# xiaolong-li1/VIDEO-BLADE

Hardware: AMD Instinct MI355X
Metric: frames/sec (aggregate over n_gpus; per GPU = value/n_gpus), CogVideoX-5B 8-step 49x720x480 bf16 (attention path); attn TFLOPS vs dense (higher is better)
Workload: dtype bf16; 1 GPU; CogVideoX-5B 8-step 49x720x480 bf16: 336 inner_attention calls per video (8 steps x 42 blocks), q/k/v [1,48,17776,64] (13x30x45 latent tokens + 226 text); global_batch=1, seq_len=17776, heads=48, head_dim=64, mask=energy rule (reference defaults), parallelism=replicas x1 (prompt-batch DP, no collective)

## Files before the change

include/vblade.h:

```cpp
#ifndef VBLADE_H_
#define VBLADE_H_

#include <stdint.h>

#ifdef __cplusplus
extern "C" {
#endif

#define VB_ABI_VERSION 4

#define VB_WORK_QUEUE_INTS 288

enum vb_status {
  VB_OK = 0,
  VB_ERR_INVALID = -1,
  VB_ERR_UNSUPPORTED = -2,
  VB_ERR_LAUNCH = -3
};

enum vb_dtype { VB_DTYPE_BF16 = 0, VB_DTYPE_F16 = 1 };
enum vb_mask_head_mode { VB_MASK_HEAD_PER_HEAD = 0, VB_MASK_HEAD_SHARED0 = 1 };

const char* vb_last_error(void);
int vb_abi_version(void);
// ... 71 lines not shown
int vb_mask_predict_long(const vb_predict_args* args, void* stream);

enum vb_rule_mode { VB_RULE_ENERGY = 0, VB_RULE_TOPK = 1 };
typedef struct vb_mask_rule {
  int mode;
  const int32_t* min_keep;
  const int32_t* max_keep;
  const float*   energy_threshold;
  int            init_k;
  const int32_t* init_k_bh;
  float          grow_below, shrink_below;
} vb_mask_rule;

int vb_mask_predict_rule(const vb_predict_args* args, const vb_mask_rule* rule, void* stream);

int vb_block_mask_rule(const void* po, int B, int H, int nr, int nc, const vb_mask_rule* rule,
                       float energy_threshold, int min_keep, int max_keep, int force_tail, int dtype,
                       uint8_t* mask, unsigned long long* mask_count, int32_t* rows_kept, void* stream);

int vb_sample_offsets(const float* rand_q, const float* rand_k, int rows, int n, int keep,
                      int32_t* q_off, int32_t* k_off, void* stream);

int vb_energy_mask(const void* po, int B, int H, int nr, int nc, float energy_threshold,
                   int min_keep, int max_keep, int force_tail, int dtype, uint8_t* mask,
                   unsigned long long* mask_count, void* stream);

int vb_pool_kv(const void* k, const void* v, const int64_t* k_stride, const int64_t* v_stride,
               const int32_t* rows, int B, int H, int L, int D, int gap, int dtype, void* kp,
               void* vp, void* k_r, void* v_r, void* stream);

// ... 223 lines not shown
```

video-blade_amd/csrc/vb_predict.hip:

```cpp
#include <cstdlib>

#include "vb_trace.hpp"

#ifndef VB_PRED_TRACE
#define VB_PRED_TRACE 0
#endif
#ifndef VB_PRED_STAMPS
#define VB_PRED_STAMPS 0
#endif
#if VB_PRED_TRACE
namespace vb { __device__ TraceBuf g_pred_trace; }
#define VB_TRACE_START(k) trace_start(g_pred_trace, k)
#define VB_TRACE_END() trace_end(g_pred_trace)
#endif
#if VB_PRED_STAMPS
namespace vb { __device__ unsigned long long g_pred_stamp[8]; }
#define VB_PRED_KERNEL_STAMPS 1
#endif

#include "vb_predict_kernel.hpp"

namespace vb {

__global__ void __launch_bounds__(256) topk_offsets_kernel(const float* rq, const float* rk, int rows, int n,
// ... 130 lines not shown
#endif
#if VB_PRED_STAMPS
extern "C" int vb_debug_pred_stamps(unsigned long long* out) {
  if (hipMemcpyFromSymbol(out, HIP_SYMBOL(vb::g_pred_stamp), 8 * sizeof(unsigned long long)) != hipSuccess) return -1;
  unsigned long long z[8] = {0, 0, 0, 0, 0, 0, 0, 0};
  return hipMemcpyToSymbol(HIP_SYMBOL(vb::g_pred_stamp), z, sizeof(z)) == hipSuccess ? 0 : -1;
}
#endif

extern "C" uint64_t vb_mask_predict_workspace_size(const vb_predict_args* a) {
  if (!a || a->B <= 0 || a->H <= 0 || a->L <= 0 || a->D <= 0 || a->num_keep <= 0) return 0;
  return vb::predict_ws_bytes(a->B, a->H, a->L, a->num_keep);
}

template <bool kLong>
static int mask_predict_entry(const vb_predict_args* a, void* stream, const vb_mask_rule* rule = nullptr) {
  using namespace vb;
  const std::string fn = rule ? "vb_mask_predict_rule: " : kLong ? "vb_mask_predict_long: " : "vb_mask_predict: ";
  if (!a || !a->q || !a->k || !a->q_off || !a->k_off || !a->po)
    return fail(VB_ERR_INVALID, fn + "null argument");
  if (a->B <= 0 || a->H <= 0 || a->L <= 0) return fail(VB_ERR_INVALID, fn + "bad sizes");
  if (a->block != 128 || (a->num_keep != 16 && a->num_keep != 32 && a->num_keep != 64))
    return fail(VB_ERR_UNSUPPORTED, fn + "block must be 128 and num_keep 16, 32 or 64 (got block " +
                                        std::to_string(a->block) + ", num_keep " + std::to_string(a->num_keep) + ")");
  const int nb = (a->L + a->block - 1) / a->block;
  if (nb > (kLong ? kMaxNbLong : kMaxNb)) return fail(VB_ERR_UNSUPPORTED, fn + "sequence too long");
  if (!kLong && a->L > 65535) return fail(VB_ERR_UNSUPPORTED, fn + "L must be < 65536");
  PredParams p{};
  if (rule) {
    if (a->mask_level) return fail(VB_ERR_INVALID, fn + "mask_level and a rule are exclusive");
    if (int rc = resolve_rule(rule, nb, a->min_keep, a->max_keep, fn, &p.rule)) return rc;
  } else if (a->min_keep < 1 || a->max_keep < 1) {
    return fail(VB_ERR_INVALID, fn + "keep counts must be >= 1");
// ... 30 lines not shown
    return fail(VB_ERR_INVALID, fn + "0..8 level bands with value/start/end arrays");
  if (a->mask_level) {
    if (!a->mask) return fail(VB_ERR_INVALID, fn + "mask_level needs a mask output");
    p.level = 1;
    p.lv.n = a->level_bands;
    for (int i = 0; i < a->level_bands; ++i) {
      const int val = a->level_band_value[i];
      if (val != 0 && val != 1 && val != 2 && val != 4 && val != 8)
        return fail(VB_ERR_INVALID, fn + "band values must be 0, 1, 2, 4 or 8");
      const int ia = (int)((double)nb * a->level_band_start[i]), ib = (int)((double)nb * a->level_band_end[i]);
      p.lv.value[i] = val;
      p.lv.start[i] = ia < 0 ? 0 : ia;
      p.lv.end[i] = ib > nb ? nb : ib;
    }
  }
  if (a->philox) {
    if (a->rand_q || a->rand_k) return fail(VB_ERR_INVALID, fn + "philox and rand_q/rand_k are exclusive");
    const int64_t one_pass = philox_x_only_numel();
    if (one_pass <= 0) return fail(VB_ERR_LAUNCH, fn + "cannot query the device's CU count");
    if ((int64_t)a->B * a->H * a->block > one_pass)
      return fail(VB_ERR_UNSUPPORTED, fn + "philox draws need B*H*block <= " + std::to_string(one_pass) +
                                          " (CUs x max threads per CU of this device)");
    p.philox = 1; p.philox_seed = a->philox_seed; p.philox_offset = a->philox_offset;
  }
  if (a->pool_kp) {
    if (!a->pool_v || !a->pool_vp || a->pool_gap <= 0 || ((a->pool_k_r == nullptr) != (a->pool_v_r == nullptr)))
      return fail(VB_ERR_INVALID, fn + "pool_v, pool_vp, pool_gap > 0 and both or neither of pool_k_r/pool_v_r");
    PoolTask& t = p.pool;
    t.D = a->D; t.gap = a->pool_gap;
    t.Lp = (a->L + a->pool_gap - 1) / a->pool_gap;
    if (int rc = fused_pass_setup(a, fn, t.Lp, t, &p.n_pool)) return rc;
    t.kp = reinterpret_cast<uint8_t*>(a->pool_kp); t.vp = reinterpret_cast<uint8_t*>(a->pool_vp);
    t.k_r = reinterpret_cast<uint8_t*>(a->pool_k_r); t.v_r = reinterpret_cast<uint8_t*>(a->pool_v_r);
  }
  if (a->pyr_k) {
    if (a->pool_kp) return fail(VB_ERR_INVALID, fn + "pool_* and pyr_* are exclusive");
    if (!a->pyr_v || !a->pool_v) return fail(VB_ERR_INVALID, fn + "pyr_k needs pyr_v and pool_v");
    PyrTask& t = p.pyr;
// ... 12 lines not shown
  hipEvent_t ev = reinterpret_cast<hipEvent_t>(a->staged_event);
  if (a->dtype != VB_DTYPE_BF16 && a->dtype != VB_DTYPE_F16) return fail(VB_ERR_INVALID, fn + "unknown dtype");
  return dispatch_predict<kLong>(p, a->dtype, a->num_keep, rule != nullptr, s, ev);
}

extern "C" int vb_mask_predict(const vb_predict_args* a, void* stream) { return mask_predict_entry<false>(a, stream); }

extern "C" int vb_mask_predict_long(const vb_predict_args* a, void* stream) {
  return mask_predict_entry<true>(a, stream);
}

extern "C" int vb_mask_predict_rule(const vb_predict_args* a, const vb_mask_rule* rule, void* stream) {
  if (rule) return mask_predict_entry<true>(a, stream, rule);
  if (a && a->block > 0 && a->L > 0 && (a->L + a->block - 1) / a->block > vb::kMaxNb) return mask_predict_entry<true>(a, stream);
  return mask_predict_entry<false>(a, stream);
}

extern "C" int vb_block_mask_rule(const void* po, int B, int H, int nr, int nc, const vb_mask_rule* rule,
                                  float energy_threshold, int min_keep, int max_keep, int force_tail, int dtype,
                                  uint8_t* mask, unsigned long long* mask_count, int32_t* rows_kept, void* stream) {
  using namespace vb;
  const std::string fn = "vb_block_mask_rule: ";
  if (!po || !mask) return fail(VB_ERR_INVALID, fn + "null argument");
  if (B <= 0 || H <= 0 || nr <= 0 || nc <= 0) return fail(VB_ERR_INVALID, fn + "bad sizes");
  if (nc > kMaxNbLong) return fail(VB_ERR_UNSUPPORTED, fn + "too many columns");
  if (force_tail < 0) return fail(VB_ERR_INVALID, fn + "force_tail must be >= 0");
  RuleParams rp{};
  vb_mask_rule none{};
  if (int rc = resolve_rule(rule ? rule : &none, nc, min_keep, max_keep, fn, &rp)) return rc;
  if (dtype != VB_DTYPE_BF16 && dtype != VB_DTYPE_F16) return fail(VB_ERR_INVALID, fn + "unknown dtype");
// ... 45 lines not shown
```

video-blade_amd/csrc/vb_predict_kernel.hpp:

```cpp
#pragma once
#include <type_traits>

#include <rocrand/rocrand_kernel.h>

#include "vb_tiles.hpp"
#include "vb_pool.hpp"
#include "vb_pyr.hpp"
#include "vb_mask_rows.hpp"

namespace vb {

constexpr int kPWaves = 4;
constexpr int kPThreads = 64 * kPWaves;
constexpr int kPMinWg = 2;
template <int D> constexpr int kKeysPerTile = (D == 64) ? 128 : 64;
template <int D> constexpr int kPBufs = D == 64 ? 2 : 3;

constexpr int kPSched = 4;
constexpr int kPRCols = 3;
typedef int i32x4 __attribute__((ext_vector_type(4)));
template <int D> constexpr bool kPoolLast = D == 128;
constexpr int kFusedPoolWgs = 320;
constexpr int kFusedPoolWgs64 = 384;

struct PredParams {
  const void* q; const void* k;
  int64_t qs[3], ks[3];
  void* reserved;
  int32_t* k_row_off;
  uint16_t* rbuf;
  const int32_t* rows;
  int32_t* q_off; int32_t* k_off;
  const float* rand_q; const float* rand_k;
  int philox; unsigned long long philox_seed, philox_offset;
  PoolTask pool;
  PyrTask pyr;
  int n_pool, pool_kind;
  int level;
  PredBands lv;
  int B, H, L, D, block, nb;
  float c;
  float thr;
  int min_keep, max_keep, force_tail;
  void* po;
  uint8_t* mask;
  unsigned long long* count;
  int32_t* rows_kept;
  int dbg;
  RuleParams rule;
};

#ifndef VB_DIAG
#define VB_DIAG 0
#endif
#ifndef VB_TRACE_START
#define VB_TRACE_START(k)
#define VB_TRACE_END()
#endif
#ifndef VB_PRED_KERNEL_STAMPS
#define VB_PRED_KERNEL_STAMPS 0
#endif
#if VB_PRED_KERNEL_STAMPS
__device__ __forceinline__ unsigned long long pred_stamp() {
  unsigned long long t;
// ... 50 lines not shown
      const float4 w = s4[j4];
      const int j = 4 * j4;
      rank += (w.x > v || (w.x == v && j < i)) ? 1 : 0;
      rank += (w.y > v || (w.y == v && j + 1 < i)) ? 1 : 0;
      rank += (w.z > v || (w.z == v && j + 2 < i)) ? 1 : 0;
      rank += (w.w > v || (w.w == v && j + 3 < i)) ? 1 : 0;
    }
    for (int j = 4 * n4; j < n; ++j) {
      const float w = sv[j];
      rank += (w > v || (w == v && j < i)) ? 1 : 0;
    }
    if (i < n && rank < keep) dst[rank] = i;
  }
}

template <class T, int kKeep = 32>
__global__ void __launch_bounds__(256) sample_rows_kernel(const PredParams p) {
  __shared__ alignas(16) float sv[2][256];
  __shared__ int32_t koff_s[kKeep];
  const int bh = blockIdx.y;
  const int wave = threadIdx.x >> 6;
  const int32_t* koff = p.k_off + (int64_t)bh * kKeep;
  if (p.philox) {
    if (wave == 0) {
      philox_draw_wave(p.philox_seed, p.philox_offset + 4, (long long)bh * p.block, p.block, sv[0]);
      topk_wave_lds(p.block, kKeep, koff_s, sv[0]);
    }
    if (blockIdx.x == 0 && wave == 1) {
      philox_draw_wave(p.philox_seed, p.philox_offset, (long long)bh * p.block, p.block, sv[1]);
      topk_wave_lds(p.block, kKeep, p.q_off + (int64_t)bh * kKeep, sv[1]);
    }
    __syncthreads();
    if (blockIdx.x == 0 && threadIdx.x < kKeep) p.k_off[(int64_t)bh * kKeep + threadIdx.x] = koff_s[threadIdx.x];
    koff = koff_s;
  } else if (p.rand_k) {
    if (wave == 0) topk_wave(p.rand_k + (int64_t)bh * p.block, p.block, kKeep, koff_s, sv[0]);
    if (blockIdx.x == 0 && wave == 1)
      topk_wave(p.rand_q + (int64_t)bh * p.block, p.block, kKeep, p.q_off + (int64_t)bh * kKeep, sv[1]);
    __syncthreads();
    if (blockIdx.x == 0 && threadIdx.x < kKeep) p.k_off[(int64_t)bh * kKeep + threadIdx.x] = koff_s[threadIdx.x];
    koff = koff_s;
  }
  const int jt = blockIdx.x * blockDim.x + threadIdx.x;
  if (jt >= p.nb * kKeep) return;
  constexpr int kKeepLog2 = kKeep == 16 ? 4 : kKeep == 32 ? 5 : 6;
  static_assert(kKeep == 1 << kKeepLog2, "sampling densities: 16, 32 or 64 tokens per block");
  int pos = min((jt >> kKeepLog2) * p.block + koff[jt & (kKeep - 1)], p.L - 1);
  if (p.rows) pos = p.rows[pos];
  p.k_row_off[(int64_t)bh * p.nb * kKeep + jt] =(int32_t)((int64_t)pos * p.ks[2] * 2);
}

template <int D, class T, bool kLong = false, int kKeep = 32, bool kRule = false>
__global__ void __launch_bounds__(kPThreads, kPMinWg) mask_predict_kernel(const PredParams p) {
  static_assert(!kRule || kLong, "the rule instantiations are long ones");
  static_assert(kKeep == 16 || kKeep == 32 || kKeep == 64, "sampling densities: 16, 32 or 64 tokens per block");
  constexpr int KS = D / 16;
  constexpr int kRowB = D * 2;
  constexpr int kKT = kKeysPerTile<D> / 32;
  constexpr int kTileBytes = kKeysPerTile<D> * kRowB;
  constexpr int kRowsPerInst = 1024 / kRowB;
  constexpr int kInstPerWave = kTileBytes / 1024 / kPWaves;
  constexpr int kBufs = kPBufs<D>;
  constexpr int KQ = 1;
  constexpr int kSt = kKeep == 16 ? kKT : KQ * (kKT / 2);
  const bool pool_wg = kPoolLast<D> ? (int)blockIdx.x >= (int)gridDim.x - p.n_pool : (int)blockIdx.x < p.n_pool;
  if (pool_wg) {
    VB_TRACE_START(1);
    const int pw = kPoolLast<D> ? (int)blockIdx.x - ((int)gridDim.x - p.n_pool) : (int)blockIdx.x;
    const int64_t i0 = (int64_t)pw * blockDim.x + threadIdx.x, st = (int64_t)p.n_pool * blockDim.x;
    if (p.pool_kind == 2) kv_pyramid_span<D, T>(p.pyr, i0, st);
    else pool_kv_span<T>(p.pool, i0, st);
    VB_TRACE_END();
    return;
  }
  VB_TRACE_START(0);
  const int wg = kPoolLast<D> ? (int)blockIdx.x : (int)blockIdx.x - p.n_pool;
  extern __shared__ __attribute__((aligned(16))) uint8_t smem[];
  const int nb = p.nb;
  float* mrow_s = reinterpret_cast<float*>(smem);
  uint8_t* ktile = smem + kPWaves * KQ * 32 * 4;
  float* rowbuf = reinterpret_cast<float*>(ktile);
  static_assert(kPWaves * 2 * kERow<kLong> * 4 <= kBufs * kTileBytes + 4 * kPWaves * 256,
                "the per-wave row scratch must fit in the K-tile ring it overlays");

  const int lane = threadIdx.x & 63;
  const int wave = __builtin_amdgcn_readfirstlane(threadIdx.x >> 6);
  const int half = lane >> 5;
  const int l32 = lane & 31;
  const int ng = kKeep == 64 ? 2 * nb : kKeep == 16 ? (nb + 1) >> 1 : nb;
  const int nqg = (ng + kPWaves * KQ - 1) / (kPWaves * KQ);
  const int lin = xcd_linear(wg, nqg * p.B * p.H);
  const int bh = lin / nqg;
// ... 319 lines not shown
  const size_t tiles = D == 64 ? (size_t)kPBufs<64> * kKeysPerTile<64> * 64 * 2
                               : (size_t)kPBufs<128> * kKeysPerTile<128> * 128 * 2;
  const size_t scratch = (size_t)kPWaves * 2 * (long_rows ? kEnergyRowLong : kEnergyRow) * 4;
  const size_t ring = 4 * kPWaves * 256;
  const size_t mrow = (size_t)kPWaves * 32 * 4;
  return mrow + (tiles + ring > scratch ? tiles + ring : scratch);
}

template <int D, class T, bool kLong, int kKeep = 32, bool kRule = false>
static int launch_predict(const PredParams& p, hipStream_t stream, hipEvent_t staged) {
  const size_t smem = predict_smem_bytes(D, kLong);
  auto kern = mask_predict_kernel<D, T, kLong, kKeep, kRule>;
  if (hipFuncSetAttribute(reinterpret_cast<const void*>(kern), hipFuncAttributeMaxDynamicSharedMemorySize,
                          (int)smem) != hipSuccess)
    return fail(VB_ERR_LAUNCH, "mask_predict: cannot reserve LDS");
  hipLaunchKernelGGL((sample_rows_kernel<T, kKeep>), dim3((unsigned)((p.nb * kKeep + 255) / 256), (unsigned)(p.B * p.H)),
                     dim3(256), 0, stream, p);
  if (int rc = check_launch("sample_rows_kernel")) return rc;
  if (staged && hipEventRecord(staged, stream) != hipSuccess) return fail(VB_ERR_LAUNCH, "vb_mask_predict: hipEventRecord failed");
  const int ng = (p.nb * kKeep + 31) / 32;
  const dim3 grid(((ng + kPWaves - 1) / kPWaves) * p.B * p.H + p.n_pool);
  hipLaunchKernelGGL(kern, grid, dim3(kPThreads), smem, stream, p);
  return check_launch("mask_predict_kernel");
}

int launch_predict_rule(const PredParams& p, int dtype, int keep, hipStream_t s, hipEvent_t ev);

}
```

video-blade_amd/vblade/_lib.py:

```python
from __future__ import annotations

import ctypes
import os

_HERE = os.path.dirname(os.path.abspath(__file__))
LIB_PATH = os.environ.get("VBLADE_LIB", os.path.join(_HERE, "libvblade_hip.so"))

VB_OK, VB_ERR_INVALID, VB_ERR_UNSUPPORTED, VB_ERR_LAUNCH = 0, -1, -2, -3
VB_DTYPE_BF16, VB_DTYPE_F16 = 0, 1

_i64x3 = ctypes.c_int64 * 3
_vp = ctypes.c_void_p
_i32p = ctypes.c_void_p


class AttnArgs(ctypes.Structure):
    _fields_ = [
        ("q", _vp), ("k", _vp), ("v", _vp),
        ("q_stride", _i64x3), ("k_stride", _i64x3), ("v_stride", _i64x3),
        ("q_rows", _vp), ("kv_rows", _vp),
        ("use_main", ctypes.c_int),
        ("block_mask", _vp), ("mask_stride", _i64x3),
        ("kp", _vp), ("vp", _vp), ("kp_stride", _i64x3), ("vp_stride", _i64x3),
        ("Lkp", ctypes.c_int), ("kp_log_bias", ctypes.c_float),
# ... 30 lines not shown
        ("mask_level", ctypes.c_int), ("level_bands", ctypes.c_int),
        ("level_band_value", _vp), ("level_band_start", _vp), ("level_band_end", _vp),
        ("mask_rows_kept", _vp),
    ]


VB_RULE_ENERGY, VB_RULE_TOPK = 0, 1


class MaskRule(ctypes.Structure):
    _fields_ = [
        ("mode", ctypes.c_int),
        ("min_keep", _vp), ("max_keep", _vp), ("energy_threshold", _vp),
        ("init_k", ctypes.c_int), ("init_k_bh", _vp),
        ("grow_below", ctypes.c_float), ("shrink_below", ctypes.c_float),
    ]


class BwdArgs(ctypes.Structure):
    _fields_ = [
        ("q", _vp), ("q_stride", _i64x3),
        ("k", _vp), ("v", _vp), ("k_stride", _i64x3), ("v_stride", _i64x3),
        ("q_rows", _vp), ("kv_rows", _vp),
        ("block_mask", _vp), ("mask_stride", _i64x3),
        ("out", _vp), ("out_stride", _i64x3),
        ("lse", _vp),
        ("kp", _vp), ("vp", _vp), ("kp_stride", _i64x3), ("vp_stride", _i64x3),
        ("Lkp", ctypes.c_int),
        ("out2", _vp), ("out2_stride", _i64x3),
        ("lse2", _vp), ("alpha", _vp),
# ... 160 lines not shown

SIGNATURES = {
    "vb_last_error": (ctypes.c_char_p, []),
    "vb_abi_version": (ctypes.c_int, []),
    "vb_gilbert3d_perm": (ctypes.c_int, [ctypes.c_int, ctypes.c_int, ctypes.c_int, _vp]),
    "vb_block_sparse_attn_fwd": (ctypes.c_int, [
        _vp, _vp, _vp, _vp, _vp, _vp, _vp, _vp,
        ctypes.c_int, ctypes.c_int, ctypes.c_int, ctypes.c_int, ctypes.c_int,
        ctypes.c_float, ctypes.c_int, ctypes.c_float, ctypes.c_int, ctypes.c_int, ctypes.c_int,
        _vp, _vp, ctypes.c_int, _vp]),
    "vb_attn_fwd": (ctypes.c_int, [ctypes.POINTER(AttnArgs), _vp]),
    "vb_mask_predict_workspace_size": (ctypes.c_uint64, [ctypes.POINTER(PredictArgs)]),
    "vb_mask_predict": (ctypes.c_int, [ctypes.POINTER(PredictArgs), _vp]),
    "vb_mask_predict_long": (ctypes.c_int, [ctypes.POINTER(PredictArgs), _vp]),
    "vb_mask_predict_rule": (ctypes.c_int, [ctypes.POINTER(PredictArgs), ctypes.POINTER(MaskRule), _vp]),
    "vb_block_mask_rule": (ctypes.c_int, [
        _vp, ctypes.c_int, ctypes.c_int, ctypes.c_int, ctypes.c_int, ctypes.POINTER(MaskRule),
        ctypes.c_float, ctypes.c_int, ctypes.c_int, ctypes.c_int, ctypes.c_int, _vp, _vp, _vp, _vp]),
    "vb_sample_offsets": (ctypes.c_int, [_vp, _vp, ctypes.c_int, ctypes.c_int, ctypes.c_int, _vp, _vp, _vp]),
    "vb_energy_mask": (ctypes.c_int, [
        _vp, ctypes.c_int, ctypes.c_int, ctypes.c_int, ctypes.c_int, ctypes.c_float,
        ctypes.c_int, ctypes.c_int, ctypes.c_int, ctypes.c_int, _vp, _vp, _vp]),
    "vb_pool_kv": (ctypes.c_int, [
        _vp, _vp, _vp, _vp, _vp, ctypes.c_int, ctypes.c_int, ctypes.c_int, ctypes.c_int,
        ctypes.c_int, ctypes.c_int, _vp, _vp, _vp, _vp, _vp]),
    "vb_attn_bwd_workspace_size": (ctypes.c_uint64, [ctypes.POINTER(BwdArgs)]),
    "vb_attn_bwd": (ctypes.c_int, [ctypes.POINTER(BwdArgs), _vp]),
    "vb_attn_bwd_joint": (ctypes.c_int, [ctypes.POINTER(BwdArgs), ctypes.c_float, _vp]),
    "vb_block_sparse_attn_bwd_workspace_size": (ctypes.c_uint64, [ctypes.c_int] * 3),
    "vb_block_sparse_attn_bwd": (ctypes.c_int, [
# ... 68 lines not shown
```

video-blade_amd/vblade/attention.py:

```python
from __future__ import annotations

from typing import Optional

import numpy as np
import torch
import torch.nn as nn

from . import ops

VARIANT_DEFAULTS = {
    "cog": dict(use_rearrange=True, max_retain_ratio=0.1, min_retain_ratio=0.05, width=45,
                height=30, depth=13, sample_gap=15, text_length=226, force_tail=2, log_every=800),
    "wan": dict(use_rearrange=True, max_retain_ratio=0.17, min_retain_ratio=0.05, width=52,
                height=30, depth=21, sample_gap=30, text_length=0, force_tail=0, log_every=200),
}


ORDER_DEFAULT = {"cog": False, "wan": True}

PERSISTENT_DEFAULT = {"cog": False, "wan": False}


def retain_counts(nb: int, min_ratio: float, max_ratio: float, variant: str):
    if variant == "cog":
        lo = int(np.float32(nb) * np.float32(min_ratio))
        hi = int(np.float32(nb) * np.float32(max_ratio))
    else:
        lo, hi = int(nb * min_ratio), int(nb * max_ratio)
    return max(1, lo), max(1, hi)


def draw_sample_offsets(B: int, H: int, device, block: int = 128, num_keep: int = 32,
                        generator: Optional[torch.Generator] = None) -> torch.Tensor:
    r = torch.rand(B, H, 1, block, device=device, generator=generator)
    return torch.topk(r, num_keep, dim=3).indices[:, :, 0, :].to(torch.int32)
# ... 71 lines not shown
    return ops.fidelity_snr_db(sums[0], sums[1]).float()


class AdaptiveBlockSparseAttn(nn.Module):

    def __init__(self, variant: str = "cog", *, combine: str = "fused", **overrides):
        super().__init__()
        if variant not in VARIANT_DEFAULTS:
            raise ValueError(f"variant must be one of {list(VARIANT_DEFAULTS)}")
        cfg = dict(VARIANT_DEFAULTS[variant])
        unknown = set(overrides) - set(cfg) - {"energy_threshold", "block", "num_keep", "overlap", "gather_kv",
                                               "mask_head_mode", "order", "order_window", "persistent",
                                               "mask_mode", "init_k", "head_budget", "judge_samples",
                                               "judge_key_stride", "judge_top", "judge_clamp", "judge_seed",
                                               "probe", "probe_samples", "probe_seed", "probe_every", "score",
                                               "grad_combine"}
        if unknown:
            raise TypeError(f"unknown options {sorted(unknown)}")
        cfg.update(overrides)
        self.variant = variant
        self.combine = combine
        self.grad_combine = cfg.get("grad_combine", "reference")
        if self.grad_combine not in ("reference", "joint"):
            raise ValueError(f"grad_combine must be 'reference' or 'joint', got {self.grad_combine!r}")
        self.use_rearrange = cfg["use_rearrange"]
        self.max_retain_ratio = cfg["max_retain_ratio"]
        self.min_retain_ratio = cfg["min_retain_ratio"]
        self.sample_gap = int(cfg["sample_gap"])
        self.text_length = int(cfg["text_length"])
        self.force_tail = int(cfg["force_tail"])
        thr = cfg.get("energy_threshold", 0.95)
# ... 81 lines not shown
        if "fidelity" in self._probes:
            prow = self.gilbert_rearranger.rows[pos.long()] if self.use_rearrange else pos
            self.register_buffer("probe_rows", prow.to(torch.int32).clone(), persistent=False)
        self.sparsity_counter = 0
        self._kept_slots = None
        self._slot_totals = []
        self.last_mask: Optional[torch.Tensor] = None
        self.attn_events: Optional[list] = None
        self.attn_event_every = 1
        self._attn_launches = 0
        self.overlap = bool(cfg.get("overlap", True))
        self.gather_kv = cfg.get("gather_kv", "auto")
        self.order = bool(cfg.get("order", ORDER_DEFAULT[variant]))
        self.order_window = int(cfg.get("order_window", 0))
        self.persistent = bool(cfg.get("persistent", PERSISTENT_DEFAULT[variant]))

    def _rows(self, device):
        if not self.use_rearrange:
            return None
        r = self.gilbert_rearranger.rows
        if r.device != device:
            r = r.to(device)
            self.gilbert_rearranger.rows = r
        return r

    def _gather(self, D: int) -> bool:
        if self.gather_kv != "auto":
            return bool(self.gather_kv)
        return D == 128

# ... 92 lines not shown
            k0 = int(nb * self.init_k) if self.init_k < 1 else int(self.init_k)
            return ops.MaskRule(mode="topk", init_k=k0)
        per_head = {n: v for n, v in (("min_keep", self.min_retain_ratio), ("max_keep", self.max_retain_ratio),
                                      ("energy_threshold", self.energy_threshold))
                    if isinstance(v, torch.Tensor)}
        if not per_head and max_keep is None:
            return None
        names = {"min_keep": "min_retain_ratio", "max_keep": "max_retain_ratio",
                 "energy_threshold": "energy_threshold"}
        fields = {n: self._per_head(names[n], v, B, H, nb, device) for n, v in per_head.items()}
        if max_keep is not None:
            fields["max_keep"] = max_keep
        return ops.MaskRule(mode="energy", **fields)

    def predict_mask(self, q, k, q_off=None, k_off=None, count=None, staged_event=None, pool=None,
                     rows_kept=None, judge_rows=None):
        B, H, L, D = q.shape
        budget = None
        if self.head_budget == "judge":
            budget = self._judge_budget(q, k, (L + self.block - 1) // self.block, judge_rows)
        if self.score == "mass":
            if pool is not None or staged_event is not None:
                raise ValueError("score='mass': the pooled K/V pass is its own launch (ops.pool_kv); "
                                 "pool= and staged_event= belong to the max predictor's launch")
            return self._predict_mask_mass(q, k, q_off, k_off, count, rows_kept, budget)
        rand = philox = None
        if q_off is None and k_off is None:
            philox = ops.claim_rand_draws(q.device, B * H * self.block)
            if philox is None:
                rand = (torch.rand(B, H, 1, self.block, device=q.device),
                        torch.rand(B, H, 1, self.block, device=q.device))
        elif q_off is None:
            q_off = draw_sample_offsets(B, H, q.device, self.block, self.num_keep)
        elif k_off is None:
            k_off = draw_sample_offsets(B, H, q.device, self.block, self.num_keep)
        nb = (L + self.block - 1) // self.block
        rule = self._mask_rule(B, H, nb, q.device, budget)
        if rule is not None:
            thr = 0.95 if isinstance(self.energy_threshold, torch.Tensor) else self.energy_threshold
            lo, hi = retain_counts(nb, 1.0 if isinstance(self.min_retain_ratio, torch.Tensor) else self.min_retain_ratio,
                                   1.0 if isinstance(self.max_retain_ratio, torch.Tensor) else self.max_retain_ratio,
                                   self.variant)
            return ops.mask_predict(q, k, q_off, k_off, rows=self._rows(q.device), energy_threshold=thr,
                                    min_keep=lo, max_keep=hi, force_tail=self.force_tail, mask_count=count,
                                    staged_event=staged_event, rand=rand, philox=philox, pool=pool,
                                    rows_kept=rows_kept, num_keep=self.num_keep, rule=rule)
        lo, hi = retain_counts(nb, self.min_retain_ratio, self.max_retain_ratio, self.variant)
        po, mask = ops.mask_predict(q, k, q_off, k_off, rows=self._rows(q.device),
                                    energy_threshold=self.energy_threshold, min_keep=lo,
                                    max_keep=hi, force_tail=self.force_tail, mask_count=count,
                                    staged_event=staged_event, rand=rand, philox=philox,
                                    pool=pool, rows_kept=rows_kept, long_rows=nb > ops.MAX_BLOCKS,
                                    num_keep=self.num_keep)
        return po, mask

    def _predict_mask_mass(self, q, k, q_off, k_off, count, rows_kept, budget):
        B, H, L, D = q.shape
        nb = (L + self.block - 1) // self.block
        if q_off is None and k_off is None:
            q_off, k_off = draw_sample_offsets_qk(B, H, q.device, self.block, self.num_keep)
        elif q_off is None:
            q_off = draw_sample_offsets(B, H, q.device, self.block, self.num_keep)
        elif k_off is None:
            k_off = draw_sample_offsets(B, H, q.device, self.block, self.num_keep)
        po = ops.mask_scores_mass(q, k, q_off, k_off, rows=self._rows(q.device))
        rule = self._mask_rule(B, H, nb, q.device, budget)
        thr, lo_r, hi_r = self.energy_threshold, self.min_retain_ratio, self.max_retain_ratio
        if rule is not None:
# ... 22 lines not shown
        grad = torch.is_grad_enabled() and (q.requires_grad or k.requires_grad or v.requires_grad)
        fused = not grad and self.combine != "reference"
        joint = grad and self.grad_combine == "joint"
        pooled = None
        rows_kept = None
        if block_mask is None:
            ride = (fused or joint) and self.overlap and self.score == "max"
            gather = self._gather(D)
            copies = joint or not (gather and rows is not None)
            outs = ops.pool_kv_outputs(k, self.sample_gap, reordered=copies) if ride else None
            if fused and self.order and self.mask_head_mode == "per_head":
                rows_kept = torch.empty(B, H, nb, device=q.device, dtype=torch.int32)
            with torch.no_grad():
                _, mask = self.predict_mask(q.detach(), k.detach(), q_off, k_off, count,
                                            pool=(v, self.sample_gap, outs) if ride else None,
                                            rows_kept=rows_kept, judge_rows=judge_rows)
            if ride:
                pooled = outs
            elif fused or joint:
                pooled = ops.pool_kv(k, v, self.sample_gap, rows, reordered=copies)
        else:
            mask = block_mask.to(torch.uint8)
            count.add_(mask.sum())
            if joint:
                pooled = ops.pool_kv(k, v, self.sample_gap, rows, reordered=True)
            elif fused:
                gather = self._gather(D)
                pooled = ops.pool_kv(k, v, self.sample_gap, rows, reordered=not (gather and rows is not None))
        self._slot_totals.append(B * H * nb * nb)
        self.sparsity_counter += 1
        self.last_mask = mask
# ... 48 lines not shown
```

video-blade_amd/vblade/ops.py:

```python
from __future__ import annotations

import ctypes
import dataclasses
import math
import os
from typing import Optional, Union

import numpy as np
import torch

from . import _lib
from ._lib import AttnArgs, BwdArgs, MlAttnArgs, MlBwdArgs, PredictArgs, check

BLOCK = 128
NUM_KEEP_VALUES = (16, 32, 64)
MAX_BLOCKS = 320
MAX_BLOCKS_LONG = 1024


def _dtype_code(t: torch.Tensor) -> int:
    if t.dtype == torch.bfloat16:
        return _lib.VB_DTYPE_BF16
    if t.dtype == torch.float16:
        return _lib.VB_DTYPE_F16
# ... 347 lines not shown
        if isinstance(rule.min_keep, torch.Tensor):
            r.min_keep = per_head("min_keep", rule.min_keep, torch.int32)
        elif rule.min_keep is not None:
            min_keep = rule.min_keep
        if isinstance(rule.max_keep, torch.Tensor):
            r.max_keep = per_head("max_keep", rule.max_keep, torch.int32)
        elif rule.max_keep is not None:
            max_keep = rule.max_keep
        if isinstance(rule.energy_threshold, torch.Tensor):
            r.energy_threshold = per_head("energy_threshold", rule.energy_threshold, torch.float32)
        elif rule.energy_threshold is not None:
            energy_threshold = rule.energy_threshold
    return r, keep, float(energy_threshold), int(min_keep), int(max_keep)


def mask_predict(q, k, q_off=None, k_off=None, *, rows=None, energy_threshold=0.95, min_keep=1,
                 max_keep=1, force_tail=0, scale=None, mask_count=None, want_mask=True,
                 staged_event=None, rand=None, philox=None, pool=None, pyr=None, level=None,
                 rows_kept=None, long_rows=False, num_keep=None, rule=None):
    try:
        return _mask_predict(q, k, q_off, k_off, rows=rows, energy_threshold=energy_threshold,
                             min_keep=min_keep, max_keep=max_keep, force_tail=force_tail, scale=scale,
                             mask_count=mask_count, want_mask=want_mask, staged_event=staged_event,
                             rand=rand, philox=philox, pool=pool, pyr=pyr, level=level,
                             rows_kept=rows_kept, long_rows=long_rows, num_keep=num_keep, rule=rule)
    except Exception as e:
        launched = isinstance(e, _lib.VBladeError) and e.code not in (None, _lib.VB_ERR_INVALID,
                                                                      _lib.VB_ERR_UNSUPPORTED)
        if philox is not None and not launched:
            release_rand_draws(q.device, philox)
        raise


def _offset_width(q_off, k_off, num_keep, drawn: bool) -> int:
    if drawn:
        keep = 32 if num_keep is None else int(num_keep)
        if keep <= 0:
            raise ValueError(f"mask_predict: num_keep must be one of {NUM_KEEP_VALUES}, got {num_keep}")
        return keep
    if q_off is None or k_off is None:
        raise ValueError("mask_predict: give q_off and k_off, or rand= or philox=")
    if q_off.shape[-1] != k_off.shape[-1]:
        raise ValueError(f"mask_predict: q_off and k_off must have the same width, got "
                         f"{q_off.shape[-1]} and {k_off.shape[-1]}")
    if num_keep is not None and int(num_keep) != q_off.shape[-1]:
        raise ValueError(f"mask_predict: the offsets are {q_off.shape[-1]} wide, num_keep={num_keep}")
    return int(q_off.shape[-1])


def _mask_predict(q, k, q_off, k_off, *, rows, energy_threshold, min_keep, max_keep, force_tail,
                  scale, mask_count, want_mask, staged_event, rand, philox, pool, pyr, level, rows_kept,
                  long_rows=False, num_keep=None, rule=None):
    keep = _offset_width(q_off, k_off, num_keep, drawn=rand is not None or philox is not None)
    if k.shape != q.shape:
        raise ValueError(f"mask_predict: k and v must have q's shape {tuple(q.shape)}, "
                         f"got k {tuple(k.shape)}")
    dev = _require_gpu(q, k, q_off, k_off, rows, rows_kept)
    q, k = _aligned_bhld(q), _aligned_bhld(k)
    B, H, L, D = q.shape
    nb = (L + BLOCK - 1) // BLOCK
    if rows_kept is not None and (level is not None or not want_mask):
        raise ValueError("mask_predict: rows_kept is written by the energy rule only (not with level= "
                         "or want_mask=False)")
    po = torch.empty(B, H, nb, nb, device=dev, dtype=q.dtype)
    mask = torch.empty(B, H, nb, nb, device=dev, dtype=torch.uint8) if want_mask else None
    if rand is not None and philox is not None:
        raise ValueError("mask_predict: rand and philox are exclusive")
    if rand is not None or philox is not None:
        if rand is not None:
            rand_q, rand_k = (r.float().contiguous() for r in rand)
        q_off = torch.empty(B, H, keep, device=dev, dtype=torch.int32)
        k_off = torch.empty(B, H, keep, device=dev, dtype=torch.int32)
    q_off = q_off.to(torch.int32).contiguous()
    k_off = k_off.to(torch.int32).contiguous()
    rule_c = None
    if rule is not None:
        if level is not None:
            raise ValueError("mask_predict: rule and level are exclusive")
        rule_c, rule_keep, energy_threshold, min_keep, max_keep = _rule_args(
            rule, B, H, dev, energy_threshold, min_keep, max_keep)
    a = PredictArgs()
    a.q, a.k = q.data_ptr(), k.data_ptr()
    a.q_stride, a.k_stride = _s3(q), _s3(k)
# ... 1 lines not shown
    a.B, a.H, a.L, a.D, a.block, a.num_keep = B, H, L, D, BLOCK, q_off.shape[-1]
    a.scale = float(scale) if scale else 0.0
    a.energy_threshold = float(energy_threshold)
    a.min_keep, a.max_keep, a.force_tail = int(min_keep), int(max_keep), int(force_tail)
    a.po, a.mask, a.mask_count = po.data_ptr(), _ptr(mask), _ptr(mask_count)
    a.dtype = _dtype_code(q)
    lib = _lib.load()
    nbytes = int(lib.vb_mask_predict_workspace_size(ctypes.byref(a)))
    ws = torch.empty(max(nbytes, 16), device=dev, dtype=torch.uint8)
    a.workspace, a.workspace_bytes = ws.data_ptr(), nbytes
    a.staged_event = staged_event.cuda_event if staged_event is not None else None
    if rand is not None:
        if rand_q.shape[-1] != BLOCK or rand_q.numel() != B * H * BLOCK or rand_k.numel() != B * H * BLOCK:
            raise ValueError("mask_predict: rand draws must be [B,H,1,block]")
        a.rand_q, a.rand_k = rand_q.data_ptr(), rand_k.data_ptr()
    if philox is not None:
        a.philox, a.philox_seed, a.philox_offset = 1, int(philox[0]), int(philox[1])
    if pool is not None:
        v, gap, outs = pool
        v = _aligned_bhld(v)
        if v.shape != k.shape:
            raise ValueError(f"mask_predict: k and v must have q's shape {tuple(q.shape)}, "
                             f"got v {tuple(v.shape)}")
        if outs[0].shape != (B, H, (L + int(gap) - 1) // int(gap), D):
            raise ValueError("mask_predict: pool outputs must come from pool_kv_outputs(k, gap)")
        a.pool_v, a.pool_v_stride, a.pool_gap = v.data_ptr(), _s3(v), int(gap)
        a.pool_kp, a.pool_vp = outs[0].data_ptr(), outs[1].data_ptr()
        if len(outs) > 2:
            a.pool_k_r, a.pool_v_r = outs[2].data_ptr(), outs[3].data_ptr()
    if pyr is not None:
        if pool is not None:
# ... 7 lines not shown
            raise ValueError("mask_predict: pyramid outputs must come from kv_pyramid_outputs(k)")
        a.pool_v, a.pool_v_stride = v.data_ptr(), _s3(v)
        a.pyr_k, a.pyr_v = outs[0].data_ptr(), outs[1].data_ptr()
    if level is not None:
        if mask is None:
            raise ValueError("mask_predict: level needs want_mask=True")
        vals, st, en = _level_bands(level)
        a.mask_level, a.level_bands = 1, len(vals)
        a.level_band_value, a.level_band_start, a.level_band_end = (
            vals.ctypes.data, st.ctypes.data, en.ctypes.data)
    if rows_kept is not None:
        if rows_kept.dtype != torch.int32 or rows_kept.numel() != B * H * nb or not rows_kept.is_contiguous():
            raise ValueError("mask_predict: rows_kept must be contiguous int32 [B,H,nb]")
        _check_dev("mask_predict: rows_kept", rows_kept, dev)
        a.mask_rows_kept = rows_kept.data_ptr()
    if rule_c is not None:
        check(lib.vb_mask_predict_rule(ctypes.byref(a), ctypes.byref(rule_c), _stream(dev)),
              "vb_mask_predict_rule")
    elif long_rows:
        check(lib.vb_mask_predict_long(ctypes.byref(a), _stream(dev)), "vb_mask_predict_long")
    else:
        check(lib.vb_mask_predict(ctypes.byref(a), _stream(dev)), "vb_mask_predict")
    return po, mask


RAND_ONE_PASS_NUMEL = 524288
PHILOX_DRAWS = os.environ.get("VB_PHILOX_DRAWS", "1") != "0"
_ONE_PASS = {}


def rand_one_pass_numel(device) -> int:
    if not torch.cuda.is_available():
        return 0
    dev = torch.device(device)
    idx = dev.index if dev.index is not None else torch.cuda.current_device()
    n = _ONE_PASS.get(idx)
    if n is None:
# ... 743 lines not shown
```

Baseline: 153.1 frames/s.

## Precompute the next predict call's sampled-row table inside the current predict kernel

Adds a sample-ahead path that appends extra workgroups to the mask-predict kernel. These workgroups draw the next call's philox offsets and build its k-row offset table, using a seed and offset peeked from the generator. When the next call's random state matches the cached key, it reuses the prepared table and skips the separate sample_rows_kernel launch, cutting a small serial kernel from each attention call. The cost is extra workgroups and LDS use in the predict grid, double-buffered int32 tables, and a dependence on correctly predicting the next generator state; on a mismatch it falls back to normal sampling.

```diff
diff --git a/include/vblade.h b/include/vblade.h
--- a/include/vblade.h
+++ b/include/vblade.h
@@ -109,6 +109,17 @@
 
 int vb_mask_predict_rule(const vb_predict_args* args, const vb_mask_rule* rule, void* stream);
 
+typedef struct vb_sample_ahead_args {
+  uint64_t next_seed;
+  uint64_t next_offset;
+  int32_t* next_q_off;
+  int32_t* next_k_off;
+  int32_t* next_table;
+  int use_table;
+  const int32_t* table;
+} vb_sample_ahead_args;
+int vb_mask_predict_ahead(const vb_predict_args* args, const vb_sample_ahead_args* ahead, void* stream);
+
 int vb_block_mask_rule(const void* po, int B, int H, int nr, int nc, const vb_mask_rule* rule,
                        float energy_threshold, int min_keep, int max_keep, int force_tail, int dtype,
                        uint8_t* mask, unsigned long long* mask_count, int32_t* rows_kept, void* stream);
diff --git a/video-blade_amd/csrc/vb_predict.hip b/video-blade_amd/csrc/vb_predict.hip
--- a/video-blade_amd/csrc/vb_predict.hip
+++ b/video-blade_amd/csrc/vb_predict.hip
@@ -168,9 +168,11 @@
 }
 
 template <bool kLong>
-static int mask_predict_entry(const vb_predict_args* a, void* stream, const vb_mask_rule* rule = nullptr) {
+static int mask_predict_entry(const vb_predict_args* a, void* stream, const vb_mask_rule* rule = nullptr,
+                              const vb_sample_ahead_args* ahead = nullptr) {
   using namespace vb;
-  const std::string fn = rule ? "vb_mask_predict_rule: " : kLong ? "vb_mask_predict_long: " : "vb_mask_predict: ";
+  const std::string fn = ahead ? "vb_mask_predict_ahead: " : rule ? "vb_mask_predict_rule: "
+                         : kLong ? "vb_mask_predict_long: " : "vb_mask_predict: ";
   if (!a || !a->q || !a->k || !a->q_off || !a->k_off || !a->po)
     return fail(VB_ERR_INVALID, fn + "null argument");
   if (a->B <= 0 || a->H <= 0 || a->L <= 0) return fail(VB_ERR_INVALID, fn + "bad sizes");
@@ -231,14 +233,34 @@
       p.lv.end[i] = ib > nb ? nb : ib;
     }
   }
-  if (a->philox) {
-    if (a->rand_q || a->rand_k) return fail(VB_ERR_INVALID, fn + "philox and rand_q/rand_k are exclusive");
+  const bool riders = ahead && ahead->next_table;
+  if (ahead) {
+    if (ahead->use_table) {
+      if (!ahead->table) return fail(VB_ERR_INVALID, fn + "use_table needs the table");
+      if (a->philox || a->rand_q || a->rand_k)
+        return fail(VB_ERR_INVALID, fn + "use_table: q_off, k_off and the table are inputs (no philox, no rand_q/rand_k)");
+      p.k_row_off = const_cast<int32_t*>(ahead->table);
+      p.ahead.have_table = 1;
+    }
+    if (riders) {
+      if (!ahead->next_q_off || !ahead->next_k_off)
+        return fail(VB_ERR_INVALID, fn + "next_table needs next_q_off and next_k_off");
+      if (ahead->next_table == p.k_row_off || ahead->next_q_off == a->q_off || ahead->next_k_off == a->k_off)
+        return fail(VB_ERR_INVALID, fn + "the next call's buffers must not be this call's");
+      p.ahead.q_off = ahead->next_q_off; p.ahead.k_off = ahead->next_k_off; p.ahead.k_row_off = ahead->next_table;
+      p.ahead.seed = ahead->next_seed; p.ahead.offset = ahead->next_offset;
+      const int bh = a->B * a->H < kAheadWgsMax ? a->B * a->H : kAheadWgsMax;
+      p.ahead.n = (bh + 7) / 8 * 8;
+    }
+  }
+  if (a->philox || riders) {
+    if (a->philox && (a->rand_q || a->rand_k)) return fail(VB_ERR_INVALID, fn + "philox and rand_q/rand_k are exclusive");
     const int64_t one_pass = philox_x_only_numel();
     if (one_pass <= 0) return fail(VB_ERR_LAUNCH, fn + "cannot query the device's CU count");
     if ((int64_t)a->B * a->H * a->block > one_pass)
       return fail(VB_ERR_UNSUPPORTED, fn + "philox draws need B*H*block <= " + std::to_string(one_pass) +
                                           " (CUs x max threads per CU of this device)");
-    p.philox = 1; p.philox_seed = a->philox_seed; p.philox_offset = a->philox_offset;
+    if (a->philox) { p.philox = 1; p.philox_seed = a->philox_seed; p.philox_offset = a->philox_offset; }
   }
   if (a->pool_kp) {
     if (!a->pool_v || !a->pool_vp || a->pool_gap <= 0 || ((a->pool_k_r == nullptr) != (a->pool_v_r == nullptr)))
@@ -281,6 +303,13 @@
   if (rule) return mask_predict_entry<true>(a, stream, rule);
   if (a && a->block > 0 && a->L > 0 && (a->L + a->block - 1) / a->block > vb::kMaxNb) return mask_predict_entry<true>(a, stream);
   return mask_predict_entry<false>(a, stream);
+}
+
+extern "C" int vb_mask_predict_ahead(const vb_predict_args* a, const vb_sample_ahead_args* ahead, void* stream) {
+  if (!ahead) return vb_mask_predict_rule(a, nullptr, stream);
+  if (a && a->block > 0 && a->L > 0 && (a->L + a->block - 1) / a->block > vb::kMaxNb)
+    return mask_predict_entry<true>(a, stream, nullptr, ahead);
+  return mask_predict_entry<false>(a, stream, nullptr, ahead);
 }
 
 extern "C" int vb_block_mask_rule(const void* po, int B, int H, int nr, int nc, const vb_mask_rule* rule,
diff --git a/video-blade_amd/csrc/vb_predict_kernel.hpp b/video-blade_amd/csrc/vb_predict_kernel.hpp
--- a/video-blade_amd/csrc/vb_predict_kernel.hpp
+++ b/video-blade_amd/csrc/vb_predict_kernel.hpp
@@ -22,6 +22,16 @@
 template <int D> constexpr bool kPoolLast = D == 128;
 constexpr int kFusedPoolWgs = 320;
 constexpr int kFusedPoolWgs64 = 384;
+template <int D> constexpr bool kAheadLast = true;
+constexpr int kAheadWgsMax = 256;
+
+struct AheadTask {
+  int32_t* q_off; int32_t* k_off;
+  int32_t* k_row_off;
+  unsigned long long seed, offset;
+  int n;
+  int have_table;
+};
 
 struct PredParams {
   const void* q; const void* k;
@@ -48,6 +58,7 @@
   int32_t* rows_kept;
   int dbg;
   RuleParams rule;
+  AheadTask ahead;
 };
 
 #ifndef VB_DIAG
@@ -128,40 +139,49 @@
   }
 }
 
+template <int kKeep>
+__device__ __forceinline__ void sample_rows_span(const PredParams& p, int philox, unsigned long long seed,
+                                                 unsigned long long offset, const float* rand_q, const float* rand_k,
+                                                 int32_t* q_off, int32_t* k_off, int32_t* k_row_off, int bh,
+                                                 int chunk, int nchunk, float* sv, int32_t* koff_s) {
+  const int wave = threadIdx.x >> 6;
+  const int32_t* koff = k_off + (int64_t)bh * kKeep;
+  if (philox) {
+    if (wave == 0) {
+      philox_draw_wave(seed, offset + 4, (long long)bh * p.block, p.block, sv);
+      topk_wave_lds(p.block, kKeep, koff_s, sv);
+    }
+    if (chunk == 0 && wave == 1) {
+      philox_draw_wave(seed, offset, (long long)bh * p.block, p.block, sv + 256);
+      topk_wave_lds(p.block, kKeep, q_off + (int64_t)bh * kKeep, sv + 256);
+    }
+    __syncthreads();
+    if (chunk == 0 && threadIdx.x < kKeep) k_off[(int64_t)bh * kKeep + threadIdx.x] = koff_s[threadIdx.x];
+    koff = koff_s;
+  } else if (rand_k) {
+    if (wave == 0) topk_wave(rand_k + (int64_t)bh * p.block, p.block, kKeep, koff_s, sv);
+    if (chunk == 0 && wave == 1)
+      topk_wave(rand_q + (int64_t)bh * p.block, p.block, kKeep, q_off + (int64_t)bh * kKeep, sv + 256);
+    __syncthreads();
+    if (chunk == 0 && threadIdx.x < kKeep) k_off[(int64_t)bh * kKeep + threadIdx.x] = koff_s[threadIdx.x];
+    koff = koff_s;
+  }
+  constexpr int kKeepLog2 = kKeep == 16 ? 4 : kKeep == 32 ? 5 : 6;
+  static_assert(kKeep == 1 << kKeepLog2, "sampling densities: 16, 32 or 64 tokens per block");
+#pragma unroll 4
+  for (int jt = chunk * (int)blockDim.x + (int)threadIdx.x; jt < p.nb * kKeep; jt += nchunk * (int)blockDim.x) {
+    int pos = min((jt >> kKeepLog2) * p.block + koff[jt & (kKeep - 1)], p.L - 1);
+    if (p.rows) pos = p.rows[pos];
+    k_row_off[(int64_t)bh * p.nb * kKeep + jt] = (int32_t)((int64_t)pos * p.ks[2] * 2);
+  }
+}
+
 template <class T, int kKeep = 32>
 __global__ void __launch_bounds__(256) sample_rows_kernel(const PredParams p) {
   __shared__ alignas(16) float sv[2][256];
   __shared__ int32_t koff_s[kKeep];
-  const int bh = blockIdx.y;
-  const int wave = threadIdx.x >> 6;
-  const int32_t* koff = p.k_off + (int64_t)bh * kKeep;
-  if (p.philox) {
-    if (wave == 0) {
-      philox_draw_wave(p.philox_seed, p.philox_offset + 4, (long long)bh * p.block, p.block, sv[0]);
-      topk_wave_lds(p.block, kKeep, koff_s, sv[0]);
-    }
-    if (blockIdx.x == 0 && wave == 1) {
-      philox_draw_wave(p.philox_seed, p.philox_offset, (long long)bh * p.block, p.block, sv[1]);
-      topk_wave_lds(p.block, kKeep, p.q_off + (int64_t)bh * kKeep, sv[1]);
-    }
-    __syncthreads();
-    if (blockIdx.x == 0 && threadIdx.x < kKeep) p.k_off[(int64_t)bh * kKeep + threadIdx.x] = koff_s[threadIdx.x];
-    koff = koff_s;
-  } else if (p.rand_k) {
-    if (wave == 0) topk_wave(p.rand_k + (int64_t)bh * p.block, p.block, kKeep, koff_s, sv[0]);
-    if (blockIdx.x == 0 && wave == 1)
-      topk_wave(p.rand_q + (int64_t)bh * p.block, p.block, kKeep, p.q_off + (int64_t)bh * kKeep, sv[1]);
-    __syncthreads();
-    if (blockIdx.x == 0 && threadIdx.x < kKeep) p.k_off[(int64_t)bh * kKeep + threadIdx.x] = koff_s[threadIdx.x];
-    koff = koff_s;
-  }
-  const int jt = blockIdx.x * blockDim.x + threadIdx.x;
-  if (jt >= p.nb * kKeep) return;
-  constexpr int kKeepLog2 = kKeep == 16 ? 4 : kKeep == 32 ? 5 : 6;
-  static_assert(kKeep == 1 << kKeepLog2, "sampling densities: 16, 32 or 64 tokens per block");
-  int pos = min((jt >> kKeepLog2) * p.block + koff[jt & (kKeep - 1)], p.L - 1);
-  if (p.rows) pos = p.rows[pos];
-  p.k_row_off[(int64_t)bh * p.nb * kKeep + jt] =(int32_t)((int64_t)pos * p.ks[2] * 2);
+  sample_rows_span<kKeep>(p, p.philox, p.philox_seed, p.philox_offset, p.rand_q, p.rand_k, p.q_off, p.k_off,
+                          p.k_row_off, blockIdx.y, blockIdx.x, gridDim.x, sv[0], koff_s);
 }
 
 template <int D, class T, bool kLong = false, int kKeep = 32, bool kRule = false>
@@ -177,10 +197,25 @@
   constexpr int kBufs = kPBufs<D>;
   constexpr int KQ = 1;
   constexpr int kSt = kKeep == 16 ? kKT : KQ * (kKT / 2);
-  const bool pool_wg = kPoolLast<D> ? (int)blockIdx.x >= (int)gridDim.x - p.n_pool : (int)blockIdx.x < p.n_pool;
+  extern __shared__ __attribute__((aligned(16))) uint8_t smem[];
+  const int gdim = (int)gridDim.x - p.ahead.n;
+  const int bx = kAheadLast<D> ? (int)blockIdx.x : (int)blockIdx.x - p.ahead.n;
+  if (kAheadLast<D> ? bx >= gdim : bx < 0) {
+    VB_TRACE_START(2);
+    float* sv = reinterpret_cast<float*>(smem);
+    int32_t* koff_s = reinterpret_cast<int32_t*>(smem + 2 * 256 * sizeof(float));
+    for (int bh = kAheadLast<D> ? bx - gdim : (int)blockIdx.x; bh < p.B * p.H; bh += p.ahead.n) {
+      sample_rows_span<kKeep>(p, 1, p.ahead.seed, p.ahead.offset, nullptr, nullptr, p.ahead.q_off, p.ahead.k_off,
+                              p.ahead.k_row_off, bh, 0, 1, sv, koff_s);
+      __syncthreads();
+    }
+    VB_TRACE_END();
+    return;
+  }
+  const bool pool_wg = kPoolLast<D> ? bx >= gdim - p.n_pool : bx < p.n_pool;
   if (pool_wg) {
     VB_TRACE_START(1);
-    const int pw = kPoolLast<D> ? (int)blockIdx.x - ((int)gridDim.x - p.n_pool) : (int)blockIdx.x;
+    const int pw = kPoolLast<D> ? bx - (gdim - p.n_pool) : bx;
     const int64_t i0 = (int64_t)pw * blockDim.x + threadIdx.x, st = (int64_t)p.n_pool * blockDim.x;
     if (p.pool_kind == 2) kv_pyramid_span<D, T>(p.pyr, i0, st);
     else pool_kv_span<T>(p.pool, i0, st);
@@ -188,8 +223,7 @@
     return;
   }
   VB_TRACE_START(0);
-  const int wg = kPoolLast<D> ? (int)blockIdx.x : (int)blockIdx.x - p.n_pool;
-  extern __shared__ __attribute__((aligned(16))) uint8_t smem[];
+  const int wg = kPoolLast<D> ? bx : bx - p.n_pool;
   const int nb = p.nb;
   float* mrow_s = reinterpret_cast<float*>(smem);
   uint8_t* ktile = smem + kPWaves * KQ * 32 * 4;
@@ -539,12 +573,14 @@
   if (hipFuncSetAttribute(reinterpret_cast<const void*>(kern), hipFuncAttributeMaxDynamicSharedMemorySize,
                           (int)smem) != hipSuccess)
     return fail(VB_ERR_LAUNCH, "mask_predict: cannot reserve LDS");
-  hipLaunchKernelGGL((sample_rows_kernel<T, kKeep>), dim3((unsigned)((p.nb * kKeep + 255) / 256), (unsigned)(p.B * p.H)),
-                     dim3(256), 0, stream, p);
-  if (int rc = check_launch("sample_rows_kernel")) return rc;
+  if (!p.ahead.have_table) {
+    hipLaunchKernelGGL((sample_rows_kernel<T, kKeep>), dim3((unsigned)((p.nb * kKeep + 255) / 256), (unsigned)(p.B * p.H)),
+                       dim3(256), 0, stream, p);
+    if (int rc = check_launch("sample_rows_kernel")) return rc;
+  }
   if (staged && hipEventRecord(staged, stream) != hipSuccess) return fail(VB_ERR_LAUNCH, "vb_mask_predict: hipEventRecord failed");
   const int ng = (p.nb * kKeep + 31) / 32;
-  const dim3 grid(((ng + kPWaves - 1) / kPWaves) * p.B * p.H + p.n_pool);
+  const dim3 grid(((ng + kPWaves - 1) / kPWaves) * p.B * p.H + p.n_pool + p.ahead.n);
   hipLaunchKernelGGL(kern, grid, dim3(kPThreads), smem, stream, p);
   return check_launch("mask_predict_kernel");
 }
diff --git a/video-blade_amd/vblade/_lib.py b/video-blade_amd/vblade/_lib.py
--- a/video-blade_amd/vblade/_lib.py
+++ b/video-blade_amd/vblade/_lib.py
@@ -68,6 +68,15 @@
         ("min_keep", _vp), ("max_keep", _vp), ("energy_threshold", _vp),
         ("init_k", ctypes.c_int), ("init_k_bh", _vp),
         ("grow_below", ctypes.c_float), ("shrink_below", ctypes.c_float),
+    ]
+
+
+class SampleAheadArgs(ctypes.Structure):
+    _fields_ = [
+        ("next_seed", ctypes.c_uint64), ("next_offset", ctypes.c_uint64),
+        ("next_q_off", _vp), ("next_k_off", _vp), ("next_table", _vp),
+        ("use_table", ctypes.c_int),
+        ("table", _vp),
     ]
 
 
@@ -258,6 +267,7 @@
     "vb_mask_predict": (ctypes.c_int, [ctypes.POINTER(PredictArgs), _vp]),
     "vb_mask_predict_long": (ctypes.c_int, [ctypes.POINTER(PredictArgs), _vp]),
     "vb_mask_predict_rule": (ctypes.c_int, [ctypes.POINTER(PredictArgs), ctypes.POINTER(MaskRule), _vp]),
+    "vb_mask_predict_ahead": (ctypes.c_int, [ctypes.POINTER(PredictArgs), ctypes.POINTER(SampleAheadArgs), _vp]),
     "vb_block_mask_rule": (ctypes.c_int, [
         _vp, ctypes.c_int, ctypes.c_int, ctypes.c_int, ctypes.c_int, ctypes.POINTER(MaskRule),
         ctypes.c_float, ctypes.c_int, ctypes.c_int, ctypes.c_int, ctypes.c_int, _vp, _vp, _vp, _vp]),
diff --git a/video-blade_amd/vblade/attention.py b/video-blade_amd/vblade/attention.py
--- a/video-blade_amd/vblade/attention.py
+++ b/video-blade_amd/vblade/attention.py
@@ -19,6 +19,8 @@
 ORDER_DEFAULT = {"cog": False, "wan": True}
 
 PERSISTENT_DEFAULT = {"cog": False, "wan": False}
+
+SAMPLE_AHEAD_DEFAULT = {"cog": True, "wan": True}
 
 
 def retain_counts(nb: int, min_ratio: float, max_ratio: float, variant: str):
@@ -120,7 +122,7 @@
                                                "mask_mode", "init_k", "head_budget", "judge_samples",
                                                "judge_key_stride", "judge_top", "judge_clamp", "judge_seed",
                                                "probe", "probe_samples", "probe_seed", "probe_every", "score",
-                                               "grad_combine"}
+                                               "grad_combine", "sample_ahead"}
         if unknown:
             raise TypeError(f"unknown options {sorted(unknown)}")
         cfg.update(overrides)
@@ -232,6 +234,12 @@
         self.order = bool(cfg.get("order", ORDER_DEFAULT[variant]))
         self.order_window = int(cfg.get("order_window", 0))
         self.persistent = bool(cfg.get("persistent", PERSISTENT_DEFAULT[variant]))
+        self.sample_ahead = bool(cfg.get("sample_ahead", SAMPLE_AHEAD_DEFAULT[variant]))
+        self._ahead = ops.SampleAhead()
+
+    @property
+    def sample_ahead_hits(self) -> int:
+        return self._ahead.hits
 
     def _rows(self, device):
         if not self.use_rearrange:
@@ -354,7 +362,7 @@
         return ops.MaskRule(mode="energy", **fields)
 
     def predict_mask(self, q, k, q_off=None, k_off=None, count=None, staged_event=None, pool=None,
-                     rows_kept=None, judge_rows=None):
+                     rows_kept=None, judge_rows=None, sample_ahead=None):
         B, H, L, D = q.shape
         budget = None
         if self.head_budget == "judge":
@@ -365,6 +373,7 @@
                                  "pool= and staged_event= belong to the max predictor's launch")
             return self._predict_mask_mass(q, k, q_off, k_off, count, rows_kept, budget)
         rand = philox = None
+        ahead = self.sample_ahead if sample_ahead is None else bool(sample_ahead)
         if q_off is None and k_off is None:
             philox = ops.claim_rand_draws(q.device, B * H * self.block)
             if philox is None:
@@ -391,7 +400,7 @@
                                     max_keep=hi, force_tail=self.force_tail, mask_count=count,
                                     staged_event=staged_event, rand=rand, philox=philox,
                                     pool=pool, rows_kept=rows_kept, long_rows=nb > ops.MAX_BLOCKS,
-                                    num_keep=self.num_keep)
+                                    num_keep=self.num_keep, ahead=self._ahead if ahead else None)
         return po, mask
 
     def _predict_mask_mass(self, q, k, q_off, k_off, count, rows_kept, budget):
@@ -444,7 +453,8 @@
             with torch.no_grad():
                 _, mask = self.predict_mask(q.detach(), k.detach(), q_off, k_off, count,
                                             pool=(v, self.sample_gap, outs) if ride else None,
-                                            rows_kept=rows_kept, judge_rows=judge_rows)
+                                            rows_kept=rows_kept, judge_rows=judge_rows,
+                                            sample_ahead=self.sample_ahead and not grad)
             if ride:
                 pooled = outs
             elif fused or joint:
diff --git a/video-blade_amd/vblade/ops.py b/video-blade_amd/vblade/ops.py
--- a/video-blade_amd/vblade/ops.py
+++ b/video-blade_amd/vblade/ops.py
@@ -385,16 +385,61 @@
     return r, keep, float(energy_threshold), int(min_keep), int(max_keep)
 
 
+class SampleAhead:
+
+    def __init__(self):
+        self.sets = None
+        self.alloc = None
+        self.cur = 0
+        self.key = None
+        self.hits = 0
+        self.calls = 0
+        self.next_state = None
+
+    @staticmethod
+    def make_key(device, stream, seed, offset, B, H, L, D, num_keep, block, k_row_stride, rows_ptr):
+        return (int(device), int(stream), int(seed), int(offset), int(B), int(H), int(L), int(D),
+                int(num_keep), int(block), int(k_row_stride), rows_ptr)
+
+    def lookup(self, key) -> bool:
+        return self.key is not None and self.key == key
+
+    def commit(self, next_key):
+        self.cur ^= 1
+        self.key = next_key
+
+    def invalidate(self):
+        self.key = None
+
+    def buffers(self, dev, stream, B, H, nb, num_keep):
+        idx = dev.index if dev.index is not None else torch.cuda.current_device()
+        alloc = (idx, int(stream), B, H, nb, num_keep)
+        if self.alloc != alloc:
+            self.sets = [(torch.empty(B, H, num_keep, device=dev, dtype=torch.int32),
+                          torch.empty(B, H, num_keep, device=dev, dtype=torch.int32),
+                          torch.empty(B, H, nb * num_keep, device=dev, dtype=torch.int32)) for _ in range(2)]
+            self.alloc, self.key, self.cur = alloc, None, 0
+        return self.sets
+
+
+def peek_rand_draws(device, generator=None):
+    if generator is None:
+        dev = torch.device(device)
+        generator = torch.cuda.default_generators[dev.index if dev.index is not None else torch.cuda.current_device()]
+    return generator.initial_seed(), generator.get_offset()
+
+
 def mask_predict(q, k, q_off=None, k_off=None, *, rows=None, energy_threshold=0.95, min_keep=1,
                  max_keep=1, force_tail=0, scale=None, mask_count=None, want_mask=True,
                  staged_event=None, rand=None, philox=None, pool=None, pyr=None, level=None,
-                 rows_kept=None, long_rows=False, num_keep=None, rule=None):
+                 rows_kept=None, long_rows=False, num_keep=None, rule=None, ahead=None, sampled=None):
     try:
         return _mask_predict(q, k, q_off, k_off, rows=rows, energy_threshold=energy_threshold,
                              min_keep=min_keep, max_keep=max_keep, force_tail=force_tail, scale=scale,
                              mask_count=mask_count, want_mask=want_mask, staged_event=staged_event,
                              rand=rand, philox=philox, pool=pool, pyr=pyr, level=level,
-                             rows_kept=rows_kept, long_rows=long_rows, num_keep=num_keep, rule=rule)
+                             rows_kept=rows_kept, long_rows=long_rows, num_keep=num_keep, rule=rule,
+                             ahead=ahead, sampled=sampled)
     except Exception as e:
         launched = isinstance(e, _lib.VBladeError) and e.code not in (None, _lib.VB_ERR_INVALID,
                                                                       _lib.VB_ERR_UNSUPPORTED)
@@ -421,7 +466,7 @@
 
 def _mask_predict(q, k, q_off, k_off, *, rows, energy_threshold, min_keep, max_keep, force_tail,
                   scale, mask_count, want_mask, staged_event, rand, philox, pool, pyr, level, rows_kept,
-                  long_rows=False, num_keep=None, rule=None):
+                  long_rows=False, num_keep=None, rule=None, ahead=None, sampled=None):
     keep = _offset_width(q_off, k_off, num_keep, drawn=rand is not None or philox is not None)
     if k.shape != q.shape:
         raise ValueError(f"mask_predict: k and v must have q's shape {tuple(q.shape)}, "
@@ -437,7 +482,26 @@
     mask = torch.empty(B, H, nb, nb, device=dev, dtype=torch.uint8) if want_mask else None
     if rand is not None and philox is not None:
         raise ValueError("mask_predict: rand and philox are exclusive")
-    if rand is not None or philox is not None:
+    ahead_c = hit_set = next_set = next_key = None
+    if ahead is not None and philox is not None and rule is None and keep in NUM_KEEP_VALUES:
+        stream = _stream(dev)
+        sets = ahead.buffers(dev, stream, B, H, nb, keep)
+        idx = dev.index if dev.index is not None else torch.cuda.current_device()
+        rows_id = None if rows is None else (rows.data_ptr(), rows._version)
+        shape = (B, H, L, D, keep, BLOCK, k.stride(2), rows_id)
+        if ahead.lookup(ahead.make_key(idx, stream, philox[0], philox[1], *shape)):
+            hit_set = sets[ahead.cur]
+        next_set = sets[ahead.cur ^ 1]
+        nseed, noff = ahead.next_state if ahead.next_state is not None else peek_rand_draws(dev)
+        next_key = ahead.make_key(idx, stream, nseed, noff, *shape)
+        ahead_c = _lib.SampleAheadArgs()
+        ahead_c.next_seed, ahead_c.next_offset = int(nseed), int(noff)
+        ahead_c.next_q_off, ahead_c.next_k_off, ahead_c.next_table = (t.data_ptr() for t in next_set)
+        ahead.invalidate()
+    if hit_set is not None:
+        q_off, k_off = hit_set[0], hit_set[1]
+        ahead_c.use_table, ahead_c.table = 1, hit_set[2].data_ptr()
+    elif rand is not None or philox is not None:
         if rand is not None:
             rand_q, rand_k = (r.float().contiguous() for r in rand)
         q_off = torch.empty(B, H, keep, device=dev, dtype=torch.int32)
@@ -469,7 +533,7 @@
         if rand_q.shape[-1] != BLOCK or rand_q.numel() != B * H * BLOCK or rand_k.numel() != B * H * BLOCK:
             raise ValueError("mask_predict: rand draws must be [B,H,1,block]")
         a.rand_q, a.rand_k = rand_q.data_ptr(), rand_k.data_ptr()
-    if philox is not None:
+    if philox is not None and hit_set is None:
         a.philox, a.philox_seed, a.philox_offset = 1, int(philox[0]), int(philox[1])
     if pool is not None:
         v, gap, outs = pool
@@ -507,13 +571,24 @@
             raise ValueError("mask_predict: rows_kept must be contiguous int32 [B,H,nb]")
         _check_dev("mask_predict: rows_kept", rows_kept, dev)
         a.mask_rows_kept = rows_kept.data_ptr()
-    if rule_c is not None:
+    if ahead_c is not None:
+        check(lib.vb_mask_predict_ahead(ctypes.byref(a), ctypes.byref(ahead_c), _stream(dev)),
+              "vb_mask_predict_ahead")
+        ahead.commit(next_key)
+        ahead.calls += 1
+        ahead.hits += hit_set is not None
+    elif rule_c is not None:
         check(lib.vb_mask_predict_rule(ctypes.byref(a), ctypes.byref(rule_c), _stream(dev)),
               "vb_mask_predict_rule")
     elif long_rows:
         check(lib.vb_mask_predict_long(ctypes.byref(a), _stream(dev)), "vb_mask_predict_long")
     else:
         check(lib.vb_mask_predict(ctypes.byref(a), _stream(dev)), "vb_mask_predict")
+    if sampled is not None:
+        table = hit_set[2] if hit_set is not None else ws[:B * H * nb * keep * 4].view(torch.int32).view(B, H, nb * keep)
+        sampled.update(q_off=q_off, k_off=k_off, table=table)
+        if next_set is not None:
+            sampled.update(next_q_off=next_set[0], next_k_off=next_set[1], next_table=next_set[2])
     return po, mask
 
 
```

Result: no change. 154.2 frames/s (median of 6 runs) (+0.8%).
